# aws/karpenter-core

Measured on AMD Instinct MI355X. Metric: pod-placement decisions/sec (Solve()), higher is better.
Workload: dtype int64

## Files before the change

karpenter_core_amd/host/encode.cpp:

```cpp
#include "encode.hpp"

#include <atomic>
#include <future>
#include <chrono>
#include <condition_variable>
#include <functional>
#include <mutex>
#include <unistd.h>
#include <exception>
#include <cstdio>
#include <cstring>
#include <sstream>
#include <string_view>
#include <thread>
#include <unordered_map>
#include <unordered_set>

namespace ksh {

namespace {

using ksp::Expr; using ksp::Pod; using ksp::StrMap;

const char* kBuiltinWellKnown[] = {ksp::kProvisionerName, ksp::kZone, ksp::kRegion, ksp::kInstanceType, ksp::kArch, ksp::kOS, ksp::kCapacityType};

struct TermRef { int type; std::string key; std::set<std::string> namespaces; ksp::Selector selector; int32_t max_skew; };

std::string selector_identity(const ksp::Selector& s) {
  if (s.nil) return "nil";
  std::string r = "sel{";
  for (auto& kv : s.match_labels) r += kv.first + "=" + kv.second + ",";
  std::vector<std::string> es;
  for (auto& e : s.match_exprs) { std::vector<std::string> vs = e.values; std::sort(vs.begin(), vs.end()); std::string x = e.key + ":" + std::to_string((int)e.op) + "["; for (auto& v : vs) x += v + ","; es.push_back(x + "]"); }
  std::sort(es.begin(), es.end()); for (auto& e : es) r += e + ";";
  return r + "}";
}

struct Filter { bool always = true; std::vector<Requirements> terms; };
Filter MakeTopologyNodeFilter(const Pod& p) {
// ... 23 lines not shown

struct Group {
  int type; std::string key; std::set<std::string> namespaces; ksp::Selector selector; int32_t max_skew; Filter filter; bool inverse; bool active;
  std::string filter_sig;
  std::map<std::string, int32_t> counts;
};

bool Relax(Pod& pod, bool toleratePreferNoSchedule) {
  if (pod.required_affinity.size() > 1) { pod.required_affinity.erase(pod.required_affinity.begin()); return true; }
  auto byw = [](const ksp::WeightedTerm& a, const ksp::WeightedTerm& b) { return a.weight > b.weight; };
  if (!pod.affinity_preferred.empty()) { std::stable_sort(pod.affinity_preferred.begin(), pod.affinity_preferred.end(), byw); pod.affinity_preferred.erase(pod.affinity_preferred.begin()); return true; }
  if (!pod.anti_preferred.empty()) { std::stable_sort(pod.anti_preferred.begin(), pod.anti_preferred.end(), byw); pod.anti_preferred.erase(pod.anti_preferred.begin()); return true; }
  if (!pod.preferred_affinity.empty()) {
    std::stable_sort(pod.preferred_affinity.begin(), pod.preferred_affinity.end(), [](const ksp::PreferredTerm& a, const ksp::PreferredTerm& b) { return a.weight > b.weight; });
    pod.preferred_affinity.erase(pod.preferred_affinity.begin()); return true;
  }
  for (size_t i = 0; i < pod.spread.size(); ++i) if (pod.spread[i].schedule_anyway) { pod.spread[i] = pod.spread.back(); pod.spread.pop_back(); return true; }
  if (toleratePreferNoSchedule) {
    for (auto& t : pod.tolerations) if (t.key.empty() && t.effect == "PreferNoSchedule" && t.op == "Exists" && t.value.empty()) return false;
    pod.tolerations.push_back({"", "Exists", "", "PreferNoSchedule"}); return true;
  }
  return false;
}

std::string canon_ip(const std::string& s) {
  int a, b, c, d; char tail;
  if (sscanf(s.c_str(), "%d.%d.%d.%d%c", &a, &b, &c, &d, &tail) == 4 && a >= 0 && a < 256 && b >= 0 && b < 256 && c >= 0 && c < 256 && d >= 0 && d < 256) { char buf[32]; snprintf(buf, sizeof buf, "%d.%d.%d.%d", a, b, c, d); return buf; }
  std::string r = s; for (auto& ch : r) ch = (char)tolower(ch);
  if (r == "0:0:0:0:0:0:0:0") r = "::";
  return r;
}

void sig_map(std::string& s, const StrMap& m) { for (auto& kv : m) { s += kv.first; s += '\1'; s += kv.second; s += '\2'; } s += '\3'; }
void sig_res(std::string& s, const ksp::ResList& r) { for (auto& kv : r) { s += kv.first; s += '\1'; s += std::to_string(kv.second); s += '\2'; } s += '\3'; }

}
uint32_t host_threads() {
  static const uint32_t n = [] {
    if (const char* e = getenv("KSH_THREADS")) { int v = atoi(e); if (v > 0) return (uint32_t)v; }
    uint32_t hw = std::max(1u, std::thread::hardware_concurrency());
    if (FILE* f = fopen("/sys/fs/cgroup/cpu.max", "r")) {
      long long period = 0; char buf[64] = {0};
      if (fscanf(f, "%63s %lld", buf, &period) == 2 && strcmp(buf, "max") != 0) { long long quota = atoll(buf); if (quota > 0 && period > 0) hw = std::min<uint32_t>(hw, (uint32_t)std::max<long long>(1, quota / period)); }
      fclose(f);
    }
    return std::min(hw, 64u);
  }();
  return n;
}
namespace {
class WorkerPool {
 public:
  static WorkerPool& get(int which) { static WorkerPool p[2]; return p[which & 1]; }
  template <class B> bool run(uint32_t n, B&& body) {
    if (n <= 1 || getpid() != pid_ || busy_.exchange(true)) return false;
    ensure(n - 1);
    std::function<void(uint32_t)> fn = [&](uint32_t t) { body(t); };
    { std::lock_guard<std::mutex> g(m_); job_ = &fn; njobs_ = n; next_ = 1; pending_ = n - 1; ++gen_; }
    cv_.notify_all();
    body(0u);
    for (;;) {
      uint32_t t; { std::lock_guard<std::mutex> g(m_); if (next_ >= njobs_) break; t = next_++; }
      body(t); { std::lock_guard<std::mutex> g(m_); --pending_; }
    }
    { std::unique_lock<std::mutex> g(m_); done_.wait(g, [&] { return pending_ == 0; }); job_ = nullptr; }
    busy_ = false; return true;
  }
// ... 63 lines not shown
  h.u(p.preferred_affinity.size()); for (auto& t : p.preferred_affinity) { h.u((uint64_t)t.weight); h.exprs(t.exprs); }
  h.u(p.tolerations.size()); for (auto& t : p.tolerations) { h.str(t.key); h.str(t.op); h.str(t.value); h.str(t.effect); }
  h.u(p.containers.size()); for (auto& c : p.containers) { h.res(c.requests); h.res(c.limits); h.u(c.ports.size()); for (auto& hp : c.ports) { h.str(hp.ip); h.u((uint64_t)hp.port); h.str(hp.proto); } }
  h.u(p.init_containers.size()); for (auto& c : p.init_containers) { h.res(c.requests); h.res(c.limits); }
  h.u(p.spread.size()); for (auto& t : p.spread) { h.u((uint64_t)t.max_skew); h.str(t.key); h.u(t.schedule_anyway); h.selector(t.selector); }
  h.u(p.affinity_required.size()); for (auto& t : p.affinity_required) h.term(t);
  h.u(p.affinity_preferred.size()); for (auto& t : p.affinity_preferred) { h.u((uint64_t)t.weight); h.term(t.term); }
  h.u(p.anti_required.size()); for (auto& t : p.anti_required) h.term(t);
  h.u(p.anti_preferred.size()); for (auto& t : p.anti_preferred) { h.u((uint64_t)t.weight); h.term(t.term); }
  h.finish(); return h;
}
bool same_exprs(const std::vector<Expr>& a, const std::vector<Expr>& b) {
  if (a.size() != b.size()) return false;
  for (size_t i = 0; i < a.size(); ++i) if (a[i].key != b[i].key || a[i].op != b[i].op || a[i].values != b[i].values) return false;
  return true;
}
bool same_selector(const ksp::Selector& a, const ksp::Selector& b) { return a.nil == b.nil && (a.nil || (a.match_labels == b.match_labels && same_exprs(a.match_exprs, b.match_exprs))); }
bool same_term(const ksp::AffinityTerm& a, const ksp::AffinityTerm& b) { return a.topology_key == b.topology_key && a.namespaces == b.namespaces && same_selector(a.selector, b.selector); }
template <class V, class F> bool same_vec(const V& a, const V& b, F&& eq) { if (a.size() != b.size()) return false; for (size_t i = 0; i < a.size(); ++i) if (!eq(a[i], b[i])) return false; return true; }
bool same_spec(const Pod& a, const Pod& b) {
  if (a.ns != b.ns || a.labels != b.labels || a.node_selector != b.node_selector) return false;
  if (!same_vec(a.required_affinity, b.required_affinity, same_exprs)) return false;
  if (!same_vec(a.preferred_affinity, b.preferred_affinity, [](const ksp::PreferredTerm& x, const ksp::PreferredTerm& y) { return x.weight == y.weight && same_exprs(x.exprs, y.exprs); })) return false;
  if (!same_vec(a.tolerations, b.tolerations, [](const ksp::Toleration& x, const ksp::Toleration& y) { return x.key == y.key && x.op == y.op && x.value == y.value && x.effect == y.effect; })) return false;
  auto same_ports = [](const ksp::HostPort& x, const ksp::HostPort& y) { return x.ip == y.ip && x.port == y.port && x.proto == y.proto; };
  if (!same_vec(a.containers, b.containers, [&](const ksp::Container& x, const ksp::Container& y) { return x.requests == y.requests && x.limits == y.limits && same_vec(x.ports, y.ports, same_ports); })) return false;
  if (!same_vec(a.init_containers, b.init_containers, [](const ksp::Container& x, const ksp::Container& y) { return x.requests == y.requests && x.limits == y.limits; })) return false;
  if (!same_vec(a.spread, b.spread, [](const ksp::Spread& x, const ksp::Spread& y) { return x.max_skew == y.max_skew && x.key == y.key && x.schedule_anyway == y.schedule_anyway && same_selector(x.selector, y.selector); })) return false;
  auto same_w = [](const ksp::WeightedTerm& x, const ksp::WeightedTerm& y) { return x.weight == y.weight && same_term(x.term, y.term); };
  return same_vec(a.affinity_required, b.affinity_required, same_term) && same_vec(a.affinity_preferred, b.affinity_preferred, same_w) &&
         same_vec(a.anti_required, b.anti_required, same_term) && same_vec(a.anti_preferred, b.anti_preferred, same_w);
}
uint64_t str_hash(std::string_view s) { Hash128 h; h.bytes(s.data(), s.size()); h.finish(); return h.a ^ h.b; }

struct Builder {
  Encoded& E; const ksp::Problem& pr; uint32_t flags;
  std::set<std::string> wellKnown;
  std::map<std::string, int> key_id; std::vector<std::set<std::string>> key_vals;
  std::vector<std::set<std::string>> key_named; std::vector<std::set<long long>> key_bounds; std::set<std::string> topo_keys; bool passive_values = false;
  std::map<std::string, int> res_id;
  std::map<std::string, int> taint_id;
  std::map<std::string, uint32_t> ip_id, proto_id;
  std::map<std::string, std::set<std::string>> domains;
  std::map<std::string, int> hostname_to_existing;
  std::map<std::string, int> hostname_to_node;
  std::vector<int> existing_row;
  std::vector<uint8_t> node_owned;
  bool any_volume_limits = false;
  int existing_of_hostname(const std::string& h) const {
    if (base) { auto it = base->hostname_to_node.find(h); return it == base->hostname_to_node.end() ? -1 : existing_row[it->second]; }
    auto it = hostname_to_existing.find(h); return it == hostname_to_existing.end() ? -1 : it->second;
  }
  const ksp::StateNode* node_named(const std::string& n) const {
    const auto& m = base ? base->node_by_name : node_by_name; auto it = m.find(n); return it == m.end() ? nullptr : it->second;
  }
  std::vector<std::unique_ptr<Group>> groups; std::map<std::string, int> topo_by_id, inverse_by_id;
  std::vector<int> group_order, group_remap;
  bool shared_filter_differs = false;
  std::vector<Requirement> it_reqs; std::map<std::string, int> it_state_id;
  std::vector<Requirement> it_cols; std::map<std::string, int> it_col_id;
  struct UidSet {
    const std::vector<std::string_view>* uids = nullptr; std::vector<uint32_t> tab; uint64_t mask = 0;
    bool count(const std::string& uid) const {
      if (tab.empty()) return false;
      for (uint64_t i = str_hash(uid) & mask;; i = (i + 1) & mask) { const uint32_t e = tab[i]; if (!e) return false; if ((*uids)[e - 1] == uid) return true; }
    }
// ... 486 lines not shown
      for (uint32_t m = 0; m < M; ++m) if (E.templates[m]->has_limits && E.templates[m]->name == pl->second) remaining[m] = Subtract(remaining[m], n.capacity);
    }
    base_remaining = remaining;
    for (uint32_t m = 0; m < M; ++m) {
      const auto& p = *E.templates[m];
      ksp::ResList dr; int count = 0;
      for (auto& d : pr.daemons) { Pod dp = d; if (!Tolerates(p.taints, dp)) continue; if (!tmpl_reqs[m].Compatible(NewPodRequirements(dp), wellKnown)) continue; dr = Merge(dr, RequestsForPod(d)); ++count; }
      dr["pods"] = (int64_t)count * 1000;
      uint32_t pm; res_vec(dr, E.tmpl_daemon, &pm); E.tmpl_daemon_present.push_back(pm);
      uint32_t lm = 0xFFFFFFFFu; if (p.has_limits) { lm = 0; for (auto& kv : p.limits) lm |= 1u << res_id.at(kv.first); }
      E.tmpl_limit_present.push_back(lm);
      res_vec(remaining[m], E.tmpl_remaining, nullptr);
    }
  }

  void count_domains(Group& g) {
    for (auto& cp : pr.cluster_pods) {
      if (!g.namespaces.count(cp.ns)) continue;
      if (!(g.selector.nil || SelectorMatches(g.selector, cp.labels))) continue;
      if (batch_uids.count(cp.uid)) continue;
      const ksp::StateNode* nptr = node_named(cp.node_name); if (!nptr) continue;
      const auto& node = *nptr;
      auto lt = node.labels.find(g.key); bool ok = lt != node.labels.end(); std::string domain = ok ? lt->second : "";
      if (!ok && g.key == ksp::kHostname) { domain = node.name; ok = true; }
      if (!ok) continue;
      if (!FilterMatches(g.filter, Requirements::FromLabels(node.labels), wellKnown)) continue;
      g.counts[domain]++;
    }
  }
  static std::string group_id(int type, const std::string& key, const std::set<std::string>& nss, const ksp::Selector& sel, int32_t max_skew, const Filter& f) {
    std::string id = key + "|" + std::to_string(type) + "|"; for (auto& n : nss) id += n + ","; id += "|" + selector_identity(sel) + "|" + std::to_string(max_skew) + "|" + filter_identity(f);
    return id;
  }
  int get_group(bool inverse, int type, const std::string& key, const std::set<std::string>& nss, const ksp::Selector& sel, int32_t max_skew, const Pod& owner, bool active_now) {
    Filter f; if (type == 0) f = MakeTopologyNodeFilter(owner);
    const std::string id = group_id(type, key, nss, sel, max_skew, f);
    auto& index = inverse ? inverse_by_id : topo_by_id;
    auto it = index.find(id);
    if (it != index.end()) {
      Group& g = *groups[it->second];
      if (!g.active && !active_now && g.filter_sig != filter_content(f)) throw Unsupported("late-created topology group whose node filter depends on which pod relaxes first");
      if (g.filter_sig != filter_content(f)) shared_filter_differs = true;
      return it->second;
    }
    auto g = std::make_unique<Group>(); g->type = type; g->key = key; g->namespaces = nss; g->selector = sel; g->max_skew = max_skew; g->filter = f; g->inverse = inverse; g->active = active_now;
    g->filter_sig = filter_content(f);
    const auto& doms = base ? base->domains : domains;
    auto d = doms.find(key); if (d != doms.end()) for (auto& v : d->second) g->counts[v] = 0;
    if (!inverse) count_domains(*g);
    int idx = (int)groups.size(); groups.push_back(std::move(g)); index[id] = idx; return idx;
  }
  static std::set<std::string> ns_list(const std::string& ns, const std::vector<std::string>& l) { if (l.empty()) return {ns}; return std::set<std::string>(l.begin(), l.end()); }

  struct SpecGroups { std::vector<int> own, iown; };
  SpecGroups groups_of(const Pod& p, bool active_now) {
    SpecGroups sg;
    if (!p.anti_required.empty() || !p.anti_preferred.empty())
      for (auto& t : p.anti_required) { int g = get_group(true, 2, t.topology_key, ns_list(p.ns, t.namespaces), t.selector, INT32_MAX, p, true); if (std::find(sg.iown.begin(), sg.iown.end(), g) == sg.iown.end()) sg.iown.push_back(g); }
    auto add = [&](int g) { if (std::find(sg.own.begin(), sg.own.end(), g) == sg.own.end()) sg.own.push_back(g); };
    for (auto& cs : p.spread) add(get_group(false, 0, cs.key, {p.ns}, cs.selector, cs.max_skew, p, active_now));
    for (auto& t : p.affinity_required) add(get_group(false, 1, t.topology_key, ns_list(p.ns, t.namespaces), t.selector, INT32_MAX, p, active_now));
    for (auto& w : p.affinity_preferred) add(get_group(false, 1, w.term.topology_key, ns_list(p.ns, w.term.namespaces), w.term.selector, INT32_MAX, p, active_now));
    for (auto& t : p.anti_required) add(get_group(false, 2, t.topology_key, ns_list(p.ns, t.namespaces), t.selector, INT32_MAX, p, active_now));
    for (auto& w : p.anti_preferred) add(get_group(false, 2, w.term.topology_key, ns_list(p.ns, w.term.namespaces), w.term.selector, INT32_MAX, p, active_now));
    return sg;
  }

  struct StageInfo { Pod spec; Requirements reqs; SpecGroups sg; };
  struct SpecInfo { std::vector<StageInfo> stages; std::vector<uint32_t> cls; };
  std::vector<SpecInfo> specs; std::unordered_map<std::string, int> spec_by_sig; std::vector<int> pod_spec;
  struct ClassRec { std::string sig; };
  std::unordered_map<std::string, uint32_t> class_by_sig;
  std::vector<std::pair<std::string, StrMap>> labelsets; std::map<std::string, int> labelset_id;
  std::vector<int> cls_labelset; std::vector<SpecGroups> cls_groups;

  void build_uid_table(uint32_t P, bool check_unique) {
    uint64_t cap = 64; while (cap < 4ull * P) cap <<= 1;
    batch_uids.uids = &uidv; batch_uids.mask = cap - 1; batch_uids.tab.assign(cap, 0);
    for (uint32_t i = 0; i < P; ++i) {
      uint64_t j = str_hash(uidv[i]) & batch_uids.mask;
      for (;; j = (j + 1) & batch_uids.mask) { const uint32_t e = batch_uids.tab[j]; if (!e) break; if (check_unique && uidv[e - 1] == uidv[i]) throw ksp::Error("pod UIDs must be unique (queue.go:102-108 needs a total order)"); }
      batch_uids.tab[j] = i + 1;
    }
  }
  void dedupe_specs() {
    if (lite) {
      if (base && !env_mode) throw ksp::Error("a binary pod batch cannot be a what-if over a snapshot");
      podp.resize(lite->size()); uidv.resize(lite->size());
      parallel_chunks(lite->size(), [&](size_t b, size_t e, uint32_t) { for (size_t i = b; i < e; ++i) { podp[i] = &lite->specs[lite->pod_spec[i]]; uidv[i] = lite->uid(i); } });
    } else {
      if (podp.empty() && !base) { podp.resize(pr.pods.size()); const Pod* p0 = pr.pods.data(); parallel_chunks(podp.size(), [&](size_t b, size_t e, uint32_t) { for (size_t i = b; i < e; ++i) podp[i] = p0 + i; }, 16384); }
      uidv.resize(podp.size()); parallel_chunks(podp.size(), [&](size_t b, size_t e, uint32_t) { for (size_t i = b; i < e; ++i) uidv[i] = podp[i]->uid; }, 16384);
    }
    const uint32_t P = (uint32_t)podp.size(); collect_volumes(); sublap("(start)");
    if (lite) {
      pod_spec.assign(lite->pod_spec.begin(), lite->pod_spec.end());
      if (!pr.cluster_pods.empty()) build_uid_table(P, true);
      specs.resize(lite->specs.size());
      parallel_chunks(specs.size(), [&](size_t b, size_t e, uint32_t) { for (size_t s2 = b; s2 < e; ++s2) { StageInfo st; st.spec = lite->specs[s2]; specs[s2].stages.push_back(std::move(st)); } }, 128);
      sublap("specs from the batch");
      return;
    }
    if (base && !env_mode) {
      const Pod* p0 = pr.pods.data();
      std::vector<int32_t> local(base->specs.size(), -1); std::vector<uint32_t> first; pod_spec.assign(P, -1);
      for (uint32_t i = 0; i < P; ++i) { const int bs = base->pod_spec[podp[i] - p0]; if (local[bs] < 0) { local[bs] = (int32_t)first.size(); first.push_back(i); } pod_spec[i] = local[bs]; }
      if (!pr.cluster_pods.empty()) build_uid_table(P, false);
      specs.resize(first.size());
      for (size_t s2 = 0; s2 < first.size(); ++s2) { StageInfo st; st.spec = *podp[first[s2]]; st.spec.uid.clear(); specs[s2].stages.push_back(std::move(st)); }
      sublap("specs from the snapshot");
      return;
    }
    if (prev && !pods_have_volumes && !prev->pods_have_volumes && !prev->spec_tab.empty() && prev->n_pods_built <= P && pr.cluster_pods.empty() == prev->batch_uids.tab.empty()) {
      const uint32_t P0 = (uint32_t)prev->n_pods_built;
      pod_spec.assign(prev->pod_spec.begin(), prev->pod_spec.begin() + P0); pod_spec.resize(P, -1);
      spec_first = prev->spec_first; spec_hs = prev->spec_hs; spec_tab = prev->spec_tab;
      uint64_t cap = spec_tab.size();
      if (cap < 4ull * P) {
// ... 26 lines not shown
    for (uint32_t i = 0; i < P; ++i) {
      uint64_t j = hs[i].a & (cap - 1);
      for (;; j = (j + 1) & (cap - 1)) { const int32_t sidx = tab[j]; if (sidx < 0) break; const Hash128& o = hs[first[sidx]]; if (o.a == hs[i].a && o.b == hs[i].b) { pod_spec[i] = sidx; break; } }
      if (pod_spec[i] < 0) { tab[j] = (int32_t)first.size(); pod_spec[i] = (int32_t)first.size(); first.push_back(i); }
    }
    sublap("spec table");
    if (!keep_warm_state && !tl_sync_confirm && P >= 8192 && host_threads() >= 4 && !getenv("KSH_NO_CONFIRM_SPECS") && !getenv("KSH_SYNC_CONFIRM")) {
      confirm_first = first;
      try {
        confirmer = std::async(std::launch::async, [this, P] {
          tl_pool = 1; std::atomic<bool> any{false};
          parallel_chunks(P, [&](size_t b, size_t e, uint32_t) { for (size_t i = b; i < e; ++i) { const uint32_t f = confirm_first[pod_spec[i]]; if (f != i && !same_pod(*podp[f], *podp[i])) any = true; } });
          return any.load() || getenv("KSH_TEST_CONFIRM_FAILS") != nullptr; });
      } catch (const std::system_error&) {}
    }
    std::vector<uint8_t> bad(P, 0);
    if (!confirmer.valid() && !getenv("KSH_NO_CONFIRM_SPECS")) parallel_chunks(P, [&](size_t b, size_t e, uint32_t) { for (size_t i = b; i < e; ++i) { const uint32_t f = first[pod_spec[i]]; if (f != i && !same_pod(*podp[f], *podp[i])) bad[i] = 1; } });
    for (uint32_t i = 0; i < P; ++i) if (bad[i]) {
      int found = -1; for (size_t s2 = 0; s2 < first.size() && found < 0; ++s2) if (same_pod(*podp[first[s2]], *podp[i])) found = (int)s2;
      if (found < 0) { found = (int)first.size(); first.push_back(i); }
      pod_spec[i] = found;
    }
    sublap("confirm"); specs.resize(first.size());
    if (keep_warm_state) {
      bool clean = true; for (uint32_t i = 0; i < P && clean; ++i) if (bad[i]) clean = false;
      if (clean) { spec_first = first; spec_tab = tab; spec_hs.resize(first.size()); for (size_t s2 = 0; s2 < first.size(); ++s2) spec_hs[s2] = hs[first[s2]]; }
    }
    parallel_chunks(first.size(), [&](size_t b, size_t e, uint32_t) { for (size_t s2 = b; s2 < e; ++s2) { StageInfo st; st.spec = *podp[first[s2]]; st.spec.uid.clear(); specs[s2].stages.push_back(std::move(st)); } }, 128);
  }

  void encode_pods() {
    const uint32_t P = (uint32_t)podp.size();
    if (confirmer.valid() && confirmer.get()) throw ConfirmFailed();
    std::future<void> sorter;
    if (!(base && !env_mode)) {
      spec_cm.resize(specs.size());
      parallel_chunks(specs.size(), [&](size_t b, size_t e, uint32_t) { for (size_t s2 = b; s2 < e; ++s2) { const ksp::ResList rq = RequestsForPod(specs[s2].stages[0].spec);
        auto c = rq.find("cpu"), m = rq.find("memory"); spec_cm[s2] = {c == rq.end() ? 0 : c->second, m == rq.end() ? 0 : m->second}; } }, 256);
      if (P >= 8192 && host_threads() >= 4 && !getenv("KSH_SYNC_QUEUE_SORT")) { try { sorter = std::async(std::launch::async, [this] { tl_pool = 1; queue_sort(); }); } catch (const std::system_error&) {} }
    }
    for (auto& cp : pr.cluster_pods) {
      if (cp.anti_required.empty() || batch_uids.count(cp.uid)) continue;
      const ksp::StateNode* nptr = node_named(cp.node_name); if (!nptr) continue;
      Pod dummy; dummy.ns = cp.ns;
      for (auto& t : cp.anti_required) {
        int gi = get_group(true, 2, t.topology_key, ns_list(cp.ns, t.namespaces), t.selector, INT32_MAX, dummy, true);
        auto lt = nptr->labels.find(groups[gi]->key); if (lt != nptr->labels.end()) groups[gi]->counts[lt->second]++;
      }
    }
    sublap("inverse affinities");
    parallel_chunks(specs.size(), [&](size_t b, size_t e, uint32_t) { for (size_t s2 = b; s2 < e; ++s2) {
      SpecInfo& si = specs[s2]; si.stages[0].reqs = NewPodRequirements(si.stages[0].spec);
      for (;;) {
        Pod next = si.stages.back().spec;
        if (!Relax(next, toleratePreferNoSchedule)) break;
        StageInfo st; st.spec = std::move(next); st.reqs = NewPodRequirements(st.spec);
        si.stages.push_back(std::move(st));
        if (si.stages.size() > 64) throw Unsupported("more than 64 relaxation stages");
      } } }, 64);
    sublap("requirements + chains (pool)");
    for (auto& si : specs) si.stages[0].sg = groups_of(si.stages[0].spec, true);
    sublap("pass A");
    for (auto& si : specs) for (size_t k = 1; k < si.stages.size(); ++k) si.stages[k].sg = groups_of(si.stages[k].spec, false);
    sublap("pass B");
    E.cls_hn_off.assign(1, 0); E.cls_port_off.assign(1, (uint32_t)E.ports.size()); E.cls_vol_off.assign(1, 0);
    { std::vector<size_t> soff(specs.size() + 1, 0); for (size_t s2 = 0; s2 < specs.size(); ++s2) soff[s2 + 1] = soff[s2] + specs[s2].stages.size();
      std::vector<ClassPre> pre(soff.back());
      parallel_chunks(specs.size(), [&](size_t b, size_t e, uint32_t) { for (size_t s2 = b; s2 < e; ++s2) for (size_t k = 0; k < specs[s2].stages.size(); ++k) class_pre(specs[s2].stages[k], pre[soff[s2] + k]); }, 64);
      sublap("class signatures (pool)");
      for (size_t s2 = 0; s2 < specs.size(); ++s2) for (size_t k = 0; k < specs[s2].stages.size(); ++k) specs[s2].cls.push_back(class_of(specs[s2].stages[k], pre[soff[s2] + k])); }
    sublap("classes"); E.pod_stage_off.resize((size_t)P + 1); E.pod_stage_off[0] = 0;
    for (uint32_t i = 0; i < P; ++i) E.pod_stage_off[i + 1] = E.pod_stage_off[i] + (uint32_t)specs[pod_spec[i]].cls.size();
    E.stage_cls.resize(E.pod_stage_off[P]);
    parallel_chunks(P, [&](size_t b, size_t e, uint32_t) { for (size_t i = b; i < e; ++i) { const auto& cl = specs[pod_spec[i]].cls; std::copy(cl.begin(), cl.end(), E.stage_cls.begin() + E.pod_stage_off[i]); } });
    if (base && !env_mode) {
      const Pod* p0 = pr.pods.data(); std::vector<std::pair<uint32_t, uint32_t>> k(P);
      for (uint32_t i = 0; i < P; ++i) k[i] = {base->pod_rank[podp[i] - p0], i};
      std::sort(k.begin(), k.end());
      E.queue.resize(P); for (uint32_t i = 0; i < P; ++i) E.queue[i] = k[i].second; sublap("queue from the snapshot's order");
      return;
    }
    sublap("chains");
    if (sorter.valid()) sorter.get(); else queue_sort();
    sublap("queue sort (joined)");
  }

  std::vector<std::pair<int64_t, int64_t>> spec_cm; std::vector<uint32_t> confirm_first; std::future<bool> confirmer;
  void queue_sort() {
    const uint32_t P = (uint32_t)podp.size();
    struct QKey { int64_t cpu, mem, ts; uint64_t u0, u1; uint32_t pod, ulen; };
    std::vector<QKey> keys(P);
    auto be64 = [](std::string_view s2, size_t off) { uint64_t v = 0; for (size_t j = 0; j < 8; ++j) v = (v << 8) | (off + j < s2.size() ? (unsigned char)s2[off + j] : 0u); return v; };
    parallel_chunks(P, [&](size_t b, size_t e, uint32_t) { for (size_t i = b; i < e; ++i) { const auto& cm0 = spec_cm[pod_spec[i]]; const std::string_view u = uidv[i];
      keys[i] = QKey{cm0.first, cm0.second, ts_of(i), be64(u, 0), be64(u, 8), (uint32_t)i, (uint32_t)u.size()}; } });
    auto less = [&](const QKey& a, const QKey& b) {
      if (a.cpu != b.cpu) return a.cpu > b.cpu;
      if (a.mem != b.mem) return a.mem > b.mem;
      if (a.ts != b.ts) return a.ts < b.ts;
      if (a.u0 != b.u0) return a.u0 < b.u0;
      if (a.u1 != b.u1) return a.u1 < b.u1;
      if (a.ulen <= 16 && b.ulen <= 16) return a.ulen < b.ulen;
      return uidv[a.pod] < uidv[b.pod];
    };
    bool bucketed = false;
    if (P >= 8192) {
      const std::vector<std::pair<int64_t, int64_t>>& cm = spec_cm;
      std::vector<std::pair<int64_t, int64_t>> dist(cm); std::sort(dist.begin(), dist.end(), [](auto& a, auto& b) { return a.first != b.first ? a.first > b.first : a.second > b.second; });
      dist.erase(std::unique(dist.begin(), dist.end()), dist.end());
      const size_t NB = dist.size();
      if (NB >= 2 && NB <= 4096) {
        std::vector<uint32_t> bucket_of(specs.size());
        for (size_t s2 = 0; s2 < specs.size(); ++s2) bucket_of[s2] = (uint32_t)(std::lower_bound(dist.begin(), dist.end(), cm[s2], [](auto& a, auto& b) { return a.first != b.first ? a.first > b.first : a.second > b.second; }) - dist.begin());
        std::vector<size_t> off(NB + 1, 0); for (uint32_t i = 0; i < P; ++i) ++off[bucket_of[pod_spec[i]] + 1];
        size_t biggest = 0; for (size_t b = 0; b < NB; ++b) { biggest = std::max(biggest, off[b + 1]); off[b + 1] += off[b]; }
        if (biggest <= P / 3) {
          std::vector<QKey> sorted(P); { std::vector<size_t> at(off.begin(), off.end() - 1); for (uint32_t i = 0; i < P; ++i) sorted[at[bucket_of[pod_spec[i]]]++] = keys[i]; }
          std::atomic<size_t> next{0};
          auto lessb = [&](const QKey& a, const QKey& b) {
            if (a.ts != b.ts) return a.ts < b.ts;
            if (a.u0 != b.u0) return a.u0 < b.u0;
            if (a.u1 != b.u1) return a.u1 < b.u1;
            if (a.ulen <= 16 && b.ulen <= 16) return a.ulen < b.ulen;
            return uidv[a.pod] < uidv[b.pod];
          };
          run_threads((uint32_t)std::min<size_t>(host_threads(), NB), [&](uint32_t) { for (;;) { const size_t b = next.fetch_add(1); if (b >= NB) return; std::sort(sorted.begin() + off[b], sorted.begin() + off[b + 1], lessb); } });
          keys.swap(sorted); bucketed = true;
        }
      }
    }
    if (!bucketed) {
      uint32_t nt = 1; while (nt * 2 <= host_threads() && (size_t)nt * 2 * 4096 <= P) nt *= 2;
      std::vector<size_t> cut(nt + 1); for (uint32_t t = 0; t <= nt; ++t) cut[t] = (size_t)P * t / nt;
      auto run = [&](uint32_t n, auto&& body) { run_threads(n, body); };
      run(nt, [&](uint32_t t) { std::sort(keys.begin() + cut[t], keys.begin() + cut[t + 1], less); });
      std::vector<QKey> tmp(nt > 1 ? P : 0);
      for (uint32_t w = 1; w < nt; w *= 2) {
        run(nt / (2 * w), [&](uint32_t t) { const size_t a = cut[2 * w * t], m = cut[2 * w * t + w], z = cut[2 * w * t + 2 * w]; std::merge(keys.begin() + a, keys.begin() + m, keys.begin() + m, keys.begin() + z, tmp.begin() + a, less); });
        keys.swap(tmp);
      }
    }
    { std::atomic<bool> dup{false};
      parallel_chunks(P, [&](size_t b, size_t e, uint32_t) { for (size_t i = std::max<size_t>(b, 1); i < e; ++i) if (keys[i].u0 == keys[i - 1].u0 && keys[i].u1 == keys[i - 1].u1 && keys[i].ulen == keys[i - 1].ulen && keys[i].ts == keys[i - 1].ts &&
                                                                                                                 keys[i].cpu == keys[i - 1].cpu && keys[i].mem == keys[i - 1].mem && uidv[keys[i].pod] == uidv[keys[i - 1].pod]) dup = true; });
      if (dup) throw ksp::Error("pod UIDs must be unique (queue.go:102-108 needs a total order)"); }
    E.queue.resize(P); for (uint32_t i = 0; i < P; ++i) E.queue[i] = keys[i].pod;
    if (keep_warm_state || !env_mode) { pod_rank.resize(P); for (uint32_t i = 0; i < P; ++i) pod_rank[E.queue[i]] = i; }
  }

  struct ClassPre { std::string ls, sig; ksp::ResList req; uint64_t tol = 0; std::vector<uint32_t> ve; std::vector<uint64_t> pe; };
  void class_pre(const StageInfo& st, ClassPre& o) const {
    const Pod& p = st.spec;
    o.ls = p.ns; o.ls += '\3'; sig_map(o.ls, p.labels);
    std::string& sig = o.sig; sig.reserve(256);
    for (auto& kv : st.reqs.m) { sig += kv.first; sig += '\1'; sig += kv.second.identity(); sig += '\2'; } sig += '\4';
    o.req = RequestsForPod(p); sig_res(sig, o.req);
    uint64_t tol = 0; for (size_t i = 0; i < taints.size(); ++i) { if ((int)i == blocked_taint) continue; bool ok = false; for (auto& t : p.tolerations) ok = ok || ToleratesTaint(t, taints[i]); if (ok) tol |= 1ull << i; }
    o.tol = tol;
    sig += std::to_string(tol); sig += '\4';
    if (pods_have_volumes) o.ve = vol_entries(p);
    for (auto e : o.ve) { sig += std::to_string(e); sig += ','; } sig += '\4';
  }
  uint32_t class_of(const StageInfo& st, ClassPre& pre) {
    const Pod& p = st.spec;
    int lsid; auto li = labelset_id.find(pre.ls); if (li == labelset_id.end()) { lsid = (int)labelsets.size(); labelsets.emplace_back(p.ns, p.labels); labelset_id[pre.ls] = lsid; } else lsid = li->second;
    std::string& sig = pre.sig; const ksp::ResList& req = pre.req; const uint64_t tol = pre.tol; const std::vector<uint32_t>& ve = pre.ve; std::vector<uint64_t>& pe = pre.pe;
    for (auto& c : p.containers) for (auto& hp : c.ports) if (hp.port != 0) pe.push_back(port_entry(hp.ip, hp.port, hp.proto));
    for (auto e : pe) { sig += std::to_string(e); sig += ','; } sig += '\4';
    sig += std::to_string(lsid); sig += '\4';
    for (int g : st.sg.own) { sig += std::to_string(g); sig += ','; } sig += '\4';
    for (int g : st.sg.iown) { sig += std::to_string(g); sig += ','; } sig += '\4';
    auto it = class_by_sig.find(sig); if (it != class_by_sig.end()) return it->second;
    const Requirement* hn = nullptr;
    uint32_t c = push_reqs(E.cls, st.reqs, &hn, true, true);
    uint8_t mode = 0;
    if (hn) {
      if (hn->greaterThan || hn->lessThan) throw Unsupported("Gt/Lt on kubernetes.io/hostname");
      mode = hn->complement ? 2 : 1;
      for (auto& v : hn->values) { const int e = existing_of_hostname(v); if (e >= 0) E.hn_list.push_back((uint32_t)e); }
    }
    E.cls_hn_mode.push_back(mode); E.cls_hn_off.push_back((uint32_t)E.hn_list.size());
    uint32_t pm; res_vec(req, E.cls_requests, &pm); E.cls_requests_present.push_back(pm);
    E.cls_tolerated.push_back(tol);
    for (auto e : pe) E.ports.push_back(e); E.cls_port_off.push_back((uint32_t)E.ports.size());
    for (auto e : ve) E.vol_list.push_back(e); E.cls_vol_off.push_back((uint32_t)E.vol_list.size());
    cls_labelset.push_back(lsid); cls_groups.push_back(st.sg);
    if (mode != 0) for (int g : st.sg.own) if (groups[g]->key == ksp::kHostname && groups[g]->type == 1) throw Unsupported("hostname pod-affinity combined with a hostname node selector");
    class_by_sig.emplace(std::move(sig), c);
    return c;
  }

  void collect_taints() {
    for (auto& p : pr.provisioners) taint_mask(p.taints);
    for (size_t i = 0; i < pr.nodes.size(); ++i) if (node_in_state(i) && pr.nodes[i].owned()) { taint_mask(pr.nodes[i].taints); if (over_volume_limit(pr.nodes[i])) blocked_mask(); }
  }

  void encode_groups() {
    std::vector<int> order, remap(groups.size(), -1);
    for (size_t g = 0; g < groups.size(); ++g) if (!groups[g]->inverse) order.push_back((int)g);
    const uint32_t ntopo = (uint32_t)order.size();
    for (size_t g = 0; g < groups.size(); ++g) if (groups[g]->inverse) order.push_back((int)g);
    for (size_t i = 0; i < order.size(); ++i) remap[order[i]] = (int)i;
    group_order = order; group_remap = remap;
    const uint32_t G = (uint32_t)order.size(); const uint32_t NE = (uint32_t)E.existing.size();
    E.grp_count.assign((size_t)G * 64, -1); E.grp_filter_off.assign(1, 0);
    uint32_t GH = 0;
    for (uint32_t gi = 0; gi < G; ++gi) {
      Group& g = *groups[order[gi]];
      E.grp_type.push_back((uint8_t)g.type); E.grp_max_skew.push_back(g.max_skew); E.grp_active.push_back(g.active ? 1 : 0);
      if (!g.filter.always) for (auto& t : g.filter.terms) {
        for (auto& kv : t.m) if (kv.first == ksp::kHostname) throw Unsupported("topology node filter on hostname");
        push_reqs(E.flt, t, nullptr, false, true);
      }
      E.grp_filter_off.push_back(E.flt.n);
      if (g.key == ksp::kHostname) {
        E.grp_key.push_back(KS_KEY_HOSTNAME); E.grp_hslot.push_back((int32_t)GH); ++GH;
        int32_t extra = 0; std::vector<int32_t> row(NE, g.active ? 0 : -1);
        for (auto& kv : g.counts) { const int e = existing_of_hostname(kv.first); if (e >= 0) row[e] = kv.second; else if (kv.second > 0) ++extra; }
        E.grph_count.insert(E.grph_count.end(), row.begin(), row.end()); E.grph_extra_pos.push_back(extra);
      } else {
        int k = key_id.at(g.key); E.grp_key.push_back(k); E.grp_hslot.push_back(-1);
// ... 604 lines not shown
```

Before: 913,500.

## Replace string signatures with interned IDs and hash indexes for groups and classes

Topology group lookup and pod class and labelset deduplication used to build long string signatures and look them up in std::map/unordered_map. They now use a string interner that maps strings to integer IDs, compact integer-vector identities, 128-bit hashes and open-addressing hash indexes, with full equality checks when hashes collide. Interning runs asynchronously during spec dedupe, and group refs are computed in the parallel chain stage rather than serially. This is meant to cut host-side string building and map lookups in encoding, at the cost of more code and a frozen/late interner path that adds mutex locking during parallel phases.

```diff
diff --git a/karpenter_core_amd/host/encode.cpp b/karpenter_core_amd/host/encode.cpp
--- a/karpenter_core_amd/host/encode.cpp
+++ b/karpenter_core_amd/host/encode.cpp
@@ -5,6 +5,7 @@
 #include <chrono>
 #include <condition_variable>
 #include <functional>
+#include <deque>
 #include <mutex>
 #include <unistd.h>
 #include <exception>
@@ -94,7 +95,6 @@
 }
 
 void sig_map(std::string& s, const StrMap& m) { for (auto& kv : m) { s += kv.first; s += '\1'; s += kv.second; s += '\2'; } s += '\3'; }
-void sig_res(std::string& s, const ksp::ResList& r) { for (auto& kv : r) { s += kv.first; s += '\1'; s += std::to_string(kv.second); s += '\2'; } s += '\3'; }
 
 }
 uint32_t host_threads() {
@@ -224,6 +224,43 @@
          same_vec(a.anti_required, b.anti_required, same_term) && same_vec(a.anti_preferred, b.anti_preferred, same_w);
 }
 uint64_t str_hash(std::string_view s) { Hash128 h; h.bytes(s.data(), s.size()); h.finish(); return h.a ^ h.b; }
+
+struct Interner {
+  std::deque<std::string> strs; std::vector<uint32_t> tab = std::vector<uint32_t>(1024, 0); bool frozen = false;
+  std::mutex mu; std::unordered_map<std::string, uint32_t> late;
+  uint32_t probe(std::string_view s, uint64_t h) const { const uint64_t mask = tab.size() - 1; for (uint64_t i = h & mask;; i = (i + 1) & mask) { const uint32_t e = tab[i]; if (!e) return 0; if (strs[e - 1] == s) return e; } }
+  void place(uint64_t h, uint32_t e) { const uint64_t mask = tab.size() - 1; uint64_t i = h & mask; while (tab[i]) i = (i + 1) & mask; tab[i] = e; }
+  uint32_t id(std::string_view s) {
+    const uint64_t h = str_hash(s);
+    if (const uint32_t e = probe(s, h)) return e;
+    if (frozen) { std::lock_guard<std::mutex> g(mu); auto it = late.find(std::string(s)); if (it == late.end()) it = late.emplace(std::string(s), 0x80000000u | (uint32_t)late.size()).first; return it->second; }
+    { std::lock_guard<std::mutex> g(mu); auto it = late.find(std::string(s)); if (it != late.end()) return it->second; }
+    strs.emplace_back(s);
+    if (strs.size() * 2 > tab.size()) { tab.assign(tab.size() * 2, 0); for (size_t k = 0; k < strs.size(); ++k) place(str_hash(strs[k]), (uint32_t)k + 1); }
+    else place(h, (uint32_t)strs.size());
+    return (uint32_t)strs.size();
+  }
+};
+struct HashIndex {
+  std::vector<std::pair<uint64_t, int32_t>> tab = std::vector<std::pair<uint64_t, int32_t>>(64, {0, -1}); size_t n = 0;
+  template <class Eq> int32_t find(uint64_t h, Eq&& same) const {
+    const uint64_t mask = tab.size() - 1;
+    for (uint64_t i = h & mask;; i = (i + 1) & mask) { const auto& e = tab[i]; if (e.second < 0) return -1; if (e.first == h && same(e.second)) return e.second; }
+  }
+  void place(uint64_t h, int32_t v) { const uint64_t mask = tab.size() - 1; uint64_t i = h & mask; while (tab[i].second >= 0) i = (i + 1) & mask; tab[i] = {h, v}; }
+  void add(uint64_t h, int32_t v) {
+    if (++n * 2 > tab.size()) { std::vector<std::pair<uint64_t, int32_t>> old(tab.size() * 2, {0, -1}); old.swap(tab); for (auto& e : old) if (e.second >= 0) place(e.first, e.second); }
+    place(h, v);
+  }
+};
+inline uint64_t test_hash_bits(uint64_t h) {
+#ifdef KS_TEST
+  static const int bits = [] { const char* e = getenv("KSH_TEST_CLASS_HASH_BITS"); return e ? atoi(e) : 64; }();
+  if (bits > 0 && bits < 64) h &= (1ull << bits) - 1;
+#endif
+  return h;
+}
+bool same_req(const Requirement& a, const Requirement& b) { return a.complement == b.complement && a.greaterThan == b.greaterThan && a.lessThan == b.lessThan && a.values == b.values; }
 
 struct Builder {
   Encoded& E; const ksp::Problem& pr; uint32_t flags;
@@ -776,46 +813,105 @@
     std::string id = key + "|" + std::to_string(type) + "|"; for (auto& n : nss) id += n + ","; id += "|" + selector_identity(sel) + "|" + std::to_string(max_skew) + "|" + filter_identity(f);
     return id;
   }
+  struct GroupRef {
+    bool inverse = false, always_active = false; int type = 0; const std::string* key = nullptr; std::set<std::string> nss; const ksp::Selector* sel = nullptr; int32_t max_skew = 0;
+    Filter f; std::string fsig; std::vector<uint32_t> idf; uint64_t h = 0;
+  };
+  Interner ids;
+  void idf_selector(std::vector<uint32_t>& o, const ksp::Selector& sl) {
+    if (sl.nil) { o.push_back(0); return; }
+    o.push_back(1); o.push_back((uint32_t)sl.match_labels.size());
+    for (auto& kv : sl.match_labels) { o.push_back(ids.id(kv.first)); o.push_back(ids.id(kv.second)); }
+    std::vector<std::vector<uint32_t>> es;
+    for (auto& e : sl.match_exprs) { std::vector<uint32_t> x{ids.id(e.key), (uint32_t)e.op}; for (auto& v : e.values) x.push_back(ids.id(v)); std::sort(x.begin() + 2, x.end()); es.push_back(std::move(x)); }
+    std::sort(es.begin(), es.end()); o.push_back((uint32_t)es.size());
+    for (auto& x : es) { o.push_back((uint32_t)x.size()); o.insert(o.end(), x.begin(), x.end()); }
+  }
+  GroupRef make_ref(bool inverse, int type, const std::string& key, std::set<std::string> nss, const ksp::Selector& sel, int32_t max_skew, const Pod& owner) {
+    GroupRef r; r.inverse = inverse; r.type = type; r.key = &key; r.nss = std::move(nss); r.sel = &sel; r.max_skew = max_skew;
+    if (type == 0) r.f = MakeTopologyNodeFilter(owner);
+    r.fsig = filter_content(r.f);
+    std::vector<uint32_t>& o = r.idf; o.reserve(32);
+    o.push_back(inverse ? 1u : 0u); o.push_back((uint32_t)type); o.push_back(ids.id(key)); o.push_back((uint32_t)max_skew);
+    o.push_back((uint32_t)r.nss.size()); { const size_t at = o.size(); for (auto& n : r.nss) o.push_back(ids.id(n)); std::sort(o.begin() + at, o.end()); }
+    idf_selector(o, sel);
+    if (r.f.always) o.push_back(0);
+    else {
+      std::vector<std::vector<uint32_t>> ts; for (auto& t : r.f.terms) { std::vector<uint32_t> x; for (auto& kv : t.m) x.push_back(ids.id(kv.first)); ts.push_back(std::move(x)); }
+      std::sort(ts.begin(), ts.end()); o.push_back(1); o.push_back((uint32_t)ts.size());
+      for (auto& x : ts) { o.push_back((uint32_t)x.size()); o.insert(o.end(), x.begin(), x.end()); }
+    }
+    Hash128 h; for (uint32_t w : o) h.u(w); h.finish(); r.h = test_hash_bits(h.a ^ h.b);
+    return r;
+  }
+  void intern_spec(const Pod& p) {
+    ids.id(p.ns); for (auto& kv : p.labels) { ids.id(kv.first); ids.id(kv.second); }
+    if (!p.spread.empty()) {
+      for (auto& kv : p.node_selector) ids.id(ksp::normalize_key(kv.first));
+      for (auto& t : p.required_affinity) for (auto& e : t) ids.id(ksp::normalize_key(e.key));
+    }
+    auto selector = [&](const ksp::Selector& sl) { if (sl.nil) return; for (auto& kv : sl.match_labels) { ids.id(kv.first); ids.id(kv.second); } for (auto& e : sl.match_exprs) { ids.id(e.key); for (auto& v : e.values) ids.id(v); } };
+    auto term = [&](const ksp::AffinityTerm& t) { ids.id(t.topology_key); for (auto& n : t.namespaces) ids.id(n); selector(t.selector); };
+    for (auto& cs : p.spread) { ids.id(cs.key); selector(cs.selector); }
+    for (auto& t : p.affinity_required) term(t);
+    for (auto& w : p.affinity_preferred) term(w.term);
+    for (auto& t : p.anti_required) term(t);
+    for (auto& w : p.anti_preferred) term(w.term);
+  }
+  struct GroupEnt { int g; std::vector<uint32_t> idf; };
+  std::vector<GroupEnt> group_ents; HashIndex group_index;
+  int group_for(const GroupRef& r, bool active_now) {
+    int gi;
+    const int32_t e = group_index.find(r.h, [&](int32_t i) { return group_ents[i].idf == r.idf; });
+    if (e >= 0) gi = group_ents[e].g;
+    else {
+      const std::string id = group_id(r.type, *r.key, r.nss, *r.sel, r.max_skew, r.f);
+      auto& index = r.inverse ? inverse_by_id : topo_by_id; auto it = index.find(id);
+      const bool fresh = it == index.end();
+      if (fresh) {
+        auto g = std::make_unique<Group>(); g->type = r.type; g->key = *r.key; g->namespaces = r.nss; g->selector = *r.sel; g->max_skew = r.max_skew; g->filter = r.f; g->inverse = r.inverse; g->active = active_now;
+        g->filter_sig = r.fsig;
+        const auto& doms = base ? base->domains : domains;
+        auto d = doms.find(*r.key); if (d != doms.end()) for (auto& v : d->second) g->counts[v] = 0;
+        if (!r.inverse) count_domains(*g);
+        gi = (int)groups.size(); groups.push_back(std::move(g)); index[id] = gi;
+      } else gi = it->second;
+      group_index.add(r.h, (int32_t)group_ents.size()); group_ents.push_back({gi, r.idf});
+      if (fresh) return gi;
+    }
+    Group& g = *groups[gi];
+    if (!g.active && !active_now && g.filter_sig != r.fsig) throw Unsupported("late-created topology group whose node filter depends on which pod relaxes first");
+    if (g.filter_sig != r.fsig) shared_filter_differs = true;
+    return gi;
+  }
   int get_group(bool inverse, int type, const std::string& key, const std::set<std::string>& nss, const ksp::Selector& sel, int32_t max_skew, const Pod& owner, bool active_now) {
-    Filter f; if (type == 0) f = MakeTopologyNodeFilter(owner);
-    const std::string id = group_id(type, key, nss, sel, max_skew, f);
-    auto& index = inverse ? inverse_by_id : topo_by_id;
-    auto it = index.find(id);
-    if (it != index.end()) {
-      Group& g = *groups[it->second];
-      if (!g.active && !active_now && g.filter_sig != filter_content(f)) throw Unsupported("late-created topology group whose node filter depends on which pod relaxes first");
-      if (g.filter_sig != filter_content(f)) shared_filter_differs = true;
-      return it->second;
-    }
-    auto g = std::make_unique<Group>(); g->type = type; g->key = key; g->namespaces = nss; g->selector = sel; g->max_skew = max_skew; g->filter = f; g->inverse = inverse; g->active = active_now;
-    g->filter_sig = filter_content(f);
-    const auto& doms = base ? base->domains : domains;
-    auto d = doms.find(key); if (d != doms.end()) for (auto& v : d->second) g->counts[v] = 0;
-    if (!inverse) count_domains(*g);
-    int idx = (int)groups.size(); groups.push_back(std::move(g)); index[id] = idx; return idx;
+    return group_for(make_ref(inverse, type, key, nss, sel, max_skew, owner), active_now);
   }
   static std::set<std::string> ns_list(const std::string& ns, const std::vector<std::string>& l) { if (l.empty()) return {ns}; return std::set<std::string>(l.begin(), l.end()); }
 
   struct SpecGroups { std::vector<int> own, iown; };
-  SpecGroups groups_of(const Pod& p, bool active_now) {
+  std::vector<GroupRef> group_refs(const Pod& p) {
+    std::vector<GroupRef> rs;
+    for (auto& t : p.anti_required) { rs.push_back(make_ref(true, 2, t.topology_key, ns_list(p.ns, t.namespaces), t.selector, INT32_MAX, p)); rs.back().always_active = true; }
+    for (auto& cs : p.spread) rs.push_back(make_ref(false, 0, cs.key, {p.ns}, cs.selector, cs.max_skew, p));
+    for (auto& t : p.affinity_required) rs.push_back(make_ref(false, 1, t.topology_key, ns_list(p.ns, t.namespaces), t.selector, INT32_MAX, p));
+    for (auto& w : p.affinity_preferred) rs.push_back(make_ref(false, 1, w.term.topology_key, ns_list(p.ns, w.term.namespaces), w.term.selector, INT32_MAX, p));
+    for (auto& t : p.anti_required) rs.push_back(make_ref(false, 2, t.topology_key, ns_list(p.ns, t.namespaces), t.selector, INT32_MAX, p));
+    for (auto& w : p.anti_preferred) rs.push_back(make_ref(false, 2, w.term.topology_key, ns_list(p.ns, w.term.namespaces), w.term.selector, INT32_MAX, p));
+    return rs;
+  }
+  SpecGroups groups_of(const std::vector<GroupRef>& refs, bool active_now) {
     SpecGroups sg;
-    if (!p.anti_required.empty() || !p.anti_preferred.empty())
-      for (auto& t : p.anti_required) { int g = get_group(true, 2, t.topology_key, ns_list(p.ns, t.namespaces), t.selector, INT32_MAX, p, true); if (std::find(sg.iown.begin(), sg.iown.end(), g) == sg.iown.end()) sg.iown.push_back(g); }
-    auto add = [&](int g) { if (std::find(sg.own.begin(), sg.own.end(), g) == sg.own.end()) sg.own.push_back(g); };
-    for (auto& cs : p.spread) add(get_group(false, 0, cs.key, {p.ns}, cs.selector, cs.max_skew, p, active_now));
-    for (auto& t : p.affinity_required) add(get_group(false, 1, t.topology_key, ns_list(p.ns, t.namespaces), t.selector, INT32_MAX, p, active_now));
-    for (auto& w : p.affinity_preferred) add(get_group(false, 1, w.term.topology_key, ns_list(p.ns, w.term.namespaces), w.term.selector, INT32_MAX, p, active_now));
-    for (auto& t : p.anti_required) add(get_group(false, 2, t.topology_key, ns_list(p.ns, t.namespaces), t.selector, INT32_MAX, p, active_now));
-    for (auto& w : p.anti_preferred) add(get_group(false, 2, w.term.topology_key, ns_list(p.ns, w.term.namespaces), w.term.selector, INT32_MAX, p, active_now));
+    for (auto& r : refs) { const int g = group_for(r, r.always_active || active_now); auto& l = r.inverse ? sg.iown : sg.own; if (std::find(l.begin(), l.end(), g) == l.end()) l.push_back(g); }
     return sg;
   }
 
-  struct StageInfo { Pod spec; Requirements reqs; SpecGroups sg; };
+  struct StageInfo { Pod spec; Requirements reqs; std::vector<GroupRef> grefs; SpecGroups sg; };
   struct SpecInfo { std::vector<StageInfo> stages; std::vector<uint32_t> cls; };
   std::vector<SpecInfo> specs; std::unordered_map<std::string, int> spec_by_sig; std::vector<int> pod_spec;
-  struct ClassRec { std::string sig; };
-  std::unordered_map<std::string, uint32_t> class_by_sig;
-  std::vector<std::pair<std::string, StrMap>> labelsets; std::map<std::string, int> labelset_id;
+  struct ClassPre;
+  std::vector<Hash128> cls_hash; std::vector<std::pair<const StageInfo*, const ClassPre*>> cls_made; HashIndex class_index;
+  std::vector<std::pair<std::string, StrMap>> labelsets; std::vector<std::vector<uint32_t>> labelset_idf; HashIndex labelset_index;
   std::vector<int> cls_labelset; std::vector<SpecGroups> cls_groups;
 
   void build_uid_table(uint32_t P, bool check_unique) {
@@ -828,6 +924,10 @@
     }
   }
   void dedupe_specs() {
+    dedupe_specs_body();
+    if (specs.size() >= 256 && host_threads() >= 4) { try { interning = std::async(std::launch::async, [this] { for (auto& si : specs) intern_spec(si.stages[0].spec); }); } catch (const std::system_error&) {} }
+  }
+  void dedupe_specs_body() {
     if (lite) {
       if (base && !env_mode) throw ksp::Error("a binary pod batch cannot be a what-if over a snapshot");
       podp.resize(lite->size()); uidv.resize(lite->size());
@@ -920,6 +1020,7 @@
   void encode_pods() {
     const uint32_t P = (uint32_t)podp.size();
     if (confirmer.valid() && confirmer.get()) throw ConfirmFailed();
+    if (interning.valid()) interning.get(); else for (auto& si : specs) intern_spec(si.stages[0].spec);
     std::future<void> sorter;
     if (!(base && !env_mode)) {
       spec_cm.resize(specs.size());
@@ -937,6 +1038,8 @@
       }
     }
     sublap("inverse affinities");
+    sublap("intern (joined)"); ids.frozen = true;
+    struct Thaw { Interner& i; ~Thaw() { i.frozen = false; } } thaw{ids};
     parallel_chunks(specs.size(), [&](size_t b, size_t e, uint32_t) { for (size_t s2 = b; s2 < e; ++s2) {
       SpecInfo& si = specs[s2]; si.stages[0].reqs = NewPodRequirements(si.stages[0].spec);
       for (;;) {
@@ -945,17 +1048,19 @@
         StageInfo st; st.spec = std::move(next); st.reqs = NewPodRequirements(st.spec);
         si.stages.push_back(std::move(st));
         if (si.stages.size() > 64) throw Unsupported("more than 64 relaxation stages");
-      } } }, 64);
+      }
+      for (auto& st : si.stages) st.grefs = group_refs(st.spec);
+      } }, 64);
     sublap("requirements + chains (pool)");
-    for (auto& si : specs) si.stages[0].sg = groups_of(si.stages[0].spec, true);
+    for (auto& si : specs) si.stages[0].sg = groups_of(si.stages[0].grefs, true);
     sublap("pass A");
-    for (auto& si : specs) for (size_t k = 1; k < si.stages.size(); ++k) si.stages[k].sg = groups_of(si.stages[k].spec, false);
+    for (auto& si : specs) for (size_t k = 1; k < si.stages.size(); ++k) si.stages[k].sg = groups_of(si.stages[k].grefs, false);
     sublap("pass B");
     E.cls_hn_off.assign(1, 0); E.cls_port_off.assign(1, (uint32_t)E.ports.size()); E.cls_vol_off.assign(1, 0);
     { std::vector<size_t> soff(specs.size() + 1, 0); for (size_t s2 = 0; s2 < specs.size(); ++s2) soff[s2 + 1] = soff[s2] + specs[s2].stages.size();
       std::vector<ClassPre> pre(soff.back());
       parallel_chunks(specs.size(), [&](size_t b, size_t e, uint32_t) { for (size_t s2 = b; s2 < e; ++s2) for (size_t k = 0; k < specs[s2].stages.size(); ++k) class_pre(specs[s2].stages[k], pre[soff[s2] + k]); }, 64);
-      sublap("class signatures (pool)");
+      sublap("class signatures (pool)"); ids.frozen = false;
       for (size_t s2 = 0; s2 < specs.size(); ++s2) for (size_t k = 0; k < specs[s2].stages.size(); ++k) specs[s2].cls.push_back(class_of(specs[s2].stages[k], pre[soff[s2] + k])); }
     sublap("classes"); E.pod_stage_off.resize((size_t)P + 1); E.pod_stage_off[0] = 0;
     for (uint32_t i = 0; i < P; ++i) E.pod_stage_off[i + 1] = E.pod_stage_off[i] + (uint32_t)specs[pod_spec[i]].cls.size();
@@ -973,7 +1078,7 @@
     sublap("queue sort (joined)");
   }
 
-  std::vector<std::pair<int64_t, int64_t>> spec_cm; std::vector<uint32_t> confirm_first; std::future<bool> confirmer;
+  std::vector<std::pair<int64_t, int64_t>> spec_cm; std::vector<uint32_t> confirm_first; std::future<bool> confirmer; std::future<void> interning;
   void queue_sort() {
     const uint32_t P = (uint32_t)podp.size();
     struct QKey { int64_t cpu, mem, ts; uint64_t u0, u1; uint32_t pod, ulen; };
@@ -1035,29 +1140,42 @@
     if (keep_warm_state || !env_mode) { pod_rank.resize(P); for (uint32_t i = 0; i < P; ++i) pod_rank[E.queue[i]] = i; }
   }
 
-  struct ClassPre { std::string ls, sig; ksp::ResList req; uint64_t tol = 0; std::vector<uint32_t> ve; std::vector<uint64_t> pe; };
-  void class_pre(const StageInfo& st, ClassPre& o) const {
+  struct ClassPre { Hash128 h; std::vector<uint32_t> ls; uint64_t lsh = 0; ksp::ResList req; uint64_t tol = 0; std::vector<uint32_t> ve; std::vector<uint64_t> pe; };
+  void class_pre(const StageInfo& st, ClassPre& o) {
     const Pod& p = st.spec;
-    o.ls = p.ns; o.ls += '\3'; sig_map(o.ls, p.labels);
-    std::string& sig = o.sig; sig.reserve(256);
-    for (auto& kv : st.reqs.m) { sig += kv.first; sig += '\1'; sig += kv.second.identity(); sig += '\2'; } sig += '\4';
-    o.req = RequestsForPod(p); sig_res(sig, o.req);
+    o.ls.reserve(1 + 2 * p.labels.size()); o.ls.push_back(ids.id(p.ns)); for (auto& kv : p.labels) { o.ls.push_back(ids.id(kv.first)); o.ls.push_back(ids.id(kv.second)); }
+    { Hash128 lh; for (uint32_t w : o.ls) lh.u(w); lh.finish(); o.lsh = test_hash_bits(lh.a ^ lh.b); }
+    Hash128& h = o.h;
+    h.u(st.reqs.m.size()); for (auto& kv : st.reqs.m) { const Requirement& r = kv.second; h.str(kv.first); h.u(r.complement); h.u(r.values.size()); for (auto& v : r.values) h.str(v);
+      h.u(r.greaterThan ? 1 : 0); h.u(r.greaterThan ? (uint64_t)*r.greaterThan : 0); h.u(r.lessThan ? 1 : 0); h.u(r.lessThan ? (uint64_t)*r.lessThan : 0); }
+    o.req = RequestsForPod(p); h.res(o.req);
     uint64_t tol = 0; for (size_t i = 0; i < taints.size(); ++i) { if ((int)i == blocked_taint) continue; bool ok = false; for (auto& t : p.tolerations) ok = ok || ToleratesTaint(t, taints[i]); if (ok) tol |= 1ull << i; }
-    o.tol = tol;
-    sig += std::to_string(tol); sig += '\4';
+    o.tol = tol; h.u(tol);
     if (pods_have_volumes) o.ve = vol_entries(p);
-    for (auto e : o.ve) { sig += std::to_string(e); sig += ','; } sig += '\4';
+    h.u(o.ve.size()); for (auto e : o.ve) h.u(e);
+  }
+  static bool same_reqs(const Requirements& a, const Requirements& b) {
+    if (a.m.size() != b.m.size()) return false;
+    for (auto i = a.m.begin(), j = b.m.begin(); i != a.m.end(); ++i, ++j) if (i->first != j->first || !same_req(i->second, j->second)) return false;
+    return true;
   }
   uint32_t class_of(const StageInfo& st, ClassPre& pre) {
     const Pod& p = st.spec;
-    int lsid; auto li = labelset_id.find(pre.ls); if (li == labelset_id.end()) { lsid = (int)labelsets.size(); labelsets.emplace_back(p.ns, p.labels); labelset_id[pre.ls] = lsid; } else lsid = li->second;
-    std::string& sig = pre.sig; const ksp::ResList& req = pre.req; const uint64_t tol = pre.tol; const std::vector<uint32_t>& ve = pre.ve; std::vector<uint64_t>& pe = pre.pe;
+    int lsid = labelset_index.find(pre.lsh, [&](int32_t l) { return labelset_idf[l] == pre.ls; });
+    if (lsid < 0) { lsid = (int)labelsets.size(); labelsets.emplace_back(p.ns, p.labels); labelset_idf.push_back(pre.ls); labelset_index.add(pre.lsh, lsid); }
+    const ksp::ResList& req = pre.req; const uint64_t tol = pre.tol; const std::vector<uint32_t>& ve = pre.ve; std::vector<uint64_t>& pe = pre.pe;
     for (auto& c : p.containers) for (auto& hp : c.ports) if (hp.port != 0) pe.push_back(port_entry(hp.ip, hp.port, hp.proto));
-    for (auto e : pe) { sig += std::to_string(e); sig += ','; } sig += '\4';
-    sig += std::to_string(lsid); sig += '\4';
-    for (int g : st.sg.own) { sig += std::to_string(g); sig += ','; } sig += '\4';
-    for (int g : st.sg.iown) { sig += std::to_string(g); sig += ','; } sig += '\4';
-    auto it = class_by_sig.find(sig); if (it != class_by_sig.end()) return it->second;
+    Hash128 h = pre.h;
+    h.u(pe.size()); for (auto e : pe) h.u(e);
+    h.u((uint64_t)lsid);
+    h.u(st.sg.own.size()); for (int g : st.sg.own) h.u((uint64_t)g);
+    h.u(st.sg.iown.size()); for (int g : st.sg.iown) h.u((uint64_t)g);
+    h.finish(); h.a = test_hash_bits(h.a); h.b = test_hash_bits(h.b);
+    const int32_t hit = class_index.find(h.a, [&](int32_t c) {
+      if (cls_hash[c].b != h.b || cls_labelset[c] != lsid || cls_groups[c].own != st.sg.own || cls_groups[c].iown != st.sg.iown) return false;
+      const StageInfo& s0 = *cls_made[c].first; const ClassPre& p0 = *cls_made[c].second;
+      return p0.tol == tol && p0.ve == ve && p0.pe == pe && p0.req == req && same_reqs(s0.reqs, st.reqs); });
+    if (hit >= 0) return (uint32_t)hit;
     const Requirement* hn = nullptr;
     uint32_t c = push_reqs(E.cls, st.reqs, &hn, true, true);
     uint8_t mode = 0;
@@ -1073,7 +1191,7 @@
     for (auto e : ve) E.vol_list.push_back(e); E.cls_vol_off.push_back((uint32_t)E.vol_list.size());
     cls_labelset.push_back(lsid); cls_groups.push_back(st.sg);
     if (mode != 0) for (int g : st.sg.own) if (groups[g]->key == ksp::kHostname && groups[g]->type == 1) throw Unsupported("hostname pod-affinity combined with a hostname node selector");
-    class_by_sig.emplace(std::move(sig), c);
+    cls_hash.push_back(h); cls_made.emplace_back(&st, &pre); class_index.add(h.a, (int32_t)c);
     return c;
   }
 
```

Measured after the change: 905,200. About the same (-0.9%).
